# UCSC-VLAA/CLIPA

Measured on AMD Instinct MI355X. Metric: image-text pairs/sec (whole job), full training step, higher is better.
Workload: dtype bf16

## Files before the change

clipa_amd/csrc/attention.hip:

```cpp
#include "common.h"
#include "clipa_hip.h"
#include "attention_common.h"
#include "internal_hooks.h"

namespace {

template <int NKT, int DH, bool CAUSAL>
__global__ __launch_bounds__((64 * attn_waves<NKT, DH>()), HD<DH>::WGS) void attn_fwd_kernel(AttnArgs pin) {
  constexpr int LP = NKT * 32, RB = HD<DH>::RB, KS = HD<DH>::KS, DT = HD<DH>::DT;
  extern __shared__ __attribute__((aligned(16))) char smem[];
  constexpr int HPW = WGHeads<NKT>::HPW, WPH = attn_waves<NKT, DH>() / HPW;
  const int tid = threadIdx.x, lane = tid & 63;
  const int wave_wg = __builtin_amdgcn_readfirstlane(tid >> 6);
  const int slot = wave_wg / WPH, wave = wave_wg % WPH;
  char* sK = smem + slot * (2 * LP * RB);
  char* sV = sK + LP * RB;
  constexpr bool STAGE = fwd_stages<NKT, DH>();
  char* stage = smem + HPW * (2 * LP * RB) + wave_wg * Stg<DH>::BYTES;
  const int l31 = lane & 31, hi = lane >> 5, q16 = (lane >> 4) & 1, i16 = lane & 15;
  const long nheads = (long)pin.B * pin.H;
  const long head_raw = (long)blockIdx.x * HPW + slot;
  const bool live = head_raw < nheads;
  const long head = live ? head_raw : nheads - 1;
  const int b = (int)(head / pin.H), h = (int)(head - (long)b * pin.H);
  ATTN_LOCATE_SEQUENCE
  const size_t hoff = ((size_t)row0 * p.ld_qkv + (size_t)h * DH) * 2;
  const unsigned nrec = (unsigned)((long)(p.L - 1) * p.ld_qkv * 2 + DH * 2);
  const __amdgpu_buffer_rsrc_t rsQ = make_rsrc(p.q + hoff, nrec);
  const __amdgpu_buffer_rsrc_t rsK = make_rsrc(p.k + hoff, nrec);
  const __amdgpu_buffer_rsrc_t rsV = make_rsrc(p.v + hoff, nrec);
  dma_image<DH>(rsK, sK, LP, p.ld_qkv, wave, lane, WPH);
  dma_image<DH>(rsV, sV, LP, p.ld_qkv, wave, lane, WPH);
  constexpr bool PREFETCH = !(NKT == 9 && DH == 64);
  bf16x8 fq[KS], fqn[KS];
  if (PREFETCH) load_frags<KS, DH>(rsQ, p.ld_qkv, 32 * wave + l31, hi, fqn);
  asm volatile("s_waitcnt vmcnt(0)" ::: "memory");
  __syncthreads();

  for (int qt = wave; qt < NKT; qt += WPH) {
    const int qg = 32 * qt + l31;
    if (PREFETCH) {
#pragma unroll
      for (int ks = 0; ks < KS; ++ks) fq[ks] = fqn[ks];
      if (qt + WPH < NKT) load_frags<KS, DH>(rsQ, p.ld_qkv, qg + 32 * WPH, hi, fqn);
    } else {
      load_frags<KS, DH>(rsQ, p.ld_qkv, qg, hi, fq);
    }
    f32x16 s[NKT];
#pragma unroll
    for (int kt = 0; kt < NKT; ++kt) {
#pragma unroll
      for (int r = 0; r < 16; ++r) s[kt][r] = 0.f;
      if (CAUSAL && kt > qt) continue;
#pragma unroll
      for (int ks = 0; ks < KS; ++ks)
        s[kt] = __builtin_amdgcn_mfma_f32_32x32x16_bf16(frag_direct<DH>(sK, 32 * kt, l31, hi, ks), fq[ks], s[kt], 0, 0, 0);
      if (!CAUSAL && (kt & 1)) __builtin_amdgcn_sched_barrier(0);
    }
    float inv, m2;
    softmax_rows<NKT, CAUSAL>(s, p, qt, qg, hi, inv, m2);

    f32x16 o[DT];
#pragma unroll
    for (int dt = 0; dt < DT; ++dt)
#pragma unroll
      for (int r = 0; r < 16; ++r) o[dt][r] = 0.f;
#pragma unroll
    for (int kt = 0; kt < NKT; ++kt) {
      if (CAUSAL && kt > qt) continue;
#pragma unroll
      for (int s2 = 0; s2 < 2; ++s2) {
        float pv[8];
#pragma unroll
        for (int e = 0; e < 8; ++e) pv[e] = s[kt][8 * s2 + e];
        const bf16x8 pf = pack_frag(pv);
#pragma unroll
        for (int dt = 0; dt < DT; ++dt)
          o[dt] = __builtin_amdgcn_mfma_f32_32x32x16_bf16(frag_trans<DH>(sV, 32 * kt + 16 * s2, 32 * dt, hi, q16, i16), pf, o[dt], 0, 0, 0);
      }
    }
    if constexpr (STAGE) {
      if (live) store_tile<DH>(stage, p.o, p.ld_o, row0 + 32 * qt, p.L - 32 * qt, h * DH, lane, o, inv);
      if (qg < p.L && live && p.stats && hi == 0) *(float2*)(p.stats + (stat0 + qg) * 2) = make_float2(m2, inv);
    } else if (qg < p.L && live) {
#pragma unroll
      for (int dt = 0; dt < DT; ++dt)
        store_frag_T(p.o, p.ld_o, row0 + qg, h * DH + 32 * dt, hi, o[dt], inv, DH - 32 * dt);
      if (p.stats && hi == 0) *(float2*)(p.stats + (stat0 + qg) * 2) = make_float2(m2, inv);
    }
  }
}

template <int NKT, int DH, bool CAUSAL>
__global__ __launch_bounds__((64 * attn_waves<NKT, DH>()), HD<DH>::WGS) void attn_bwd_kernel(AttnArgs pin) {
  constexpr int LP = NKT * 32, RB = HD<DH>::RB, KS = HD<DH>::KS, DT = HD<DH>::DT;
  extern __shared__ __attribute__((aligned(16))) char smem[];
  constexpr int HPW = WGHeads<NKT>::HPW, WPH = attn_waves<NKT, DH>() / HPW;
  constexpr bool FENCE = DH == 80 && NKT >= 5;
  const int tid = threadIdx.x, lane = tid & 63;
  const int wave_wg = __builtin_amdgcn_readfirstlane(tid >> 6);
  const int slot = wave_wg / WPH, wave = wave_wg % WPH;
  char* img0 = smem + slot * (2 * LP * RB + 3 * LP * 4);
  char* img1 = img0 + LP * RB;
  float* sM = (float*)(img0 + 2 * LP * RB);
  float* sD = sM + 2 * LP;
  constexpr bool STAGE = bwd_stages<NKT, DH>();
  char* stage = smem + HPW * (2 * LP * RB + 3 * LP * 4) + wave_wg * Stg<DH>::BYTES;
  const int l31 = lane & 31, hi = lane >> 5, q16 = (lane >> 4) & 1, i16 = lane & 15;
  const long nheads = (long)pin.B * pin.H;
  const long head_raw = (long)blockIdx.x * HPW + slot;
  const bool live = head_raw < nheads;
  const long head = live ? head_raw : nheads - 1;
  const int b = (int)(head / pin.H), h = (int)(head - (long)b * pin.H);
  ATTN_LOCATE_SEQUENCE
  const size_t hoff = ((size_t)row0 * p.ld_qkv + (size_t)h * DH) * 2;
  const size_t ooff = ((size_t)row0 * p.ld_o + (size_t)h * DH) * 2;
  const unsigned nrec = (unsigned)((long)(p.L - 1) * p.ld_qkv * 2 + DH * 2);
  const unsigned nrec_o = (unsigned)((long)(p.L - 1) * p.ld_o * 2 + DH * 2);
  const __amdgpu_buffer_rsrc_t rsQ = make_rsrc(p.q + hoff, nrec), rsK = make_rsrc(p.k + hoff, nrec),
                               rsV = make_rsrc(p.v + hoff, nrec), rsDO = make_rsrc(p.d_o + ooff, nrec_o),
                               rsO = make_rsrc(p.o_in + ooff, nrec_o);
  const float c = p.scale * 1.4426950408889634f;
  const float* stats = p.stats + stat0 * 2;

  dma_image<DH>(rsK, img0, LP, p.ld_qkv, wave, lane, WPH);
  dma_image<DH>(rsV, img1, LP, p.ld_qkv, wave, lane, WPH);
  bf16x8 fq[KS], fdo[KS], fo[KS];
  load_frags<KS, DH>(rsQ, p.ld_qkv, 32 * wave + l31, hi, fq);
  load_frags<KS, DH>(rsDO, p.ld_o, 32 * wave + l31, hi, fdo);
  load_frags<KS, DH>(rsO, p.ld_o, 32 * wave + l31, hi, fo);
  asm volatile("s_waitcnt vmcnt(0)" ::: "memory");
  __syncthreads();
  for (int qt = wave; qt < NKT; qt += WPH) {
    const int qg = 32 * qt + l31;
    if (qt != wave) {
      load_frags<KS, DH>(rsQ, p.ld_qkv, qg, hi, fq);
      load_frags<KS, DH>(rsDO, p.ld_o, qg, hi, fdo);
      load_frags<KS, DH>(rsO, p.ld_o, qg, hi, fo);
    }
    float mp = 1e30f;
    if (qg < p.L) {
      const float2 st = *(const float2*)(stats + qg * 2);
      mp = st.x - __builtin_amdgcn_logf(st.y);
    }
    float Dq = 0.f;
#pragma unroll
    for (int ks = 0; ks < KS; ++ks) {
      float a[8], o8[8];
      unpack8(__builtin_bit_cast(u32x4, fdo[ks]), a);
      unpack8(__builtin_bit_cast(u32x4, fo[ks]), o8);
#pragma unroll
      for (int i = 0; i < 8; ++i) Dq += a[i] * o8[i];
    }
    Dq += __shfl_xor(Dq, 32, 64);
    if (hi == 0) { sM[qg] = mp; sD[qg] = Dq; }
    const int lim2 = (CAUSAL ? min(p.L, qg + 1) : p.L) - 4 * hi;
    f32x16 dq[DT];
#pragma unroll
    for (int dt = 0; dt < DT; ++dt)
#pragma unroll
      for (int r = 0; r < 16; ++r) dq[dt][r] = 0.f;
#pragma unroll
    for (int kt = 0; kt < NKT; ++kt) {
      if (CAUSAL && kt > qt) continue;
      f32x16 s, dp;
#pragma unroll
      for (int r = 0; r < 16; ++r) { s[r] = 0.f; dp[r] = 0.f; }
#pragma unroll
      for (int ks = 0; ks < KS; ++ks) {
        s = __builtin_amdgcn_mfma_f32_32x32x16_bf16(frag_direct<DH>(img0, 32 * kt, l31, hi, ks), fq[ks], s, 0, 0, 0);
        dp = __builtin_amdgcn_mfma_f32_32x32x16_bf16(frag_direct<DH>(img1, 32 * kt, l31, hi, ks), fdo[ks], dp, 0, 0, 0);
      }
      if constexpr (FENCE) __builtin_amdgcn_sched_barrier(0);
      const bool full = CAUSAL ? ((32 * kt + 32 <= p.L) && kt < qt) : (kt < NKT - 1);
      float ds[16];
#pragma unroll
      for (int r = 0; r < 16; ++r) {
        float pe = __builtin_amdgcn_exp2f(fmaf(s[r], c, -mp));
        if (!full) pe = (32 * kt + 8 * (r >> 2) + (r & 3) < lim2) ? pe : 0.f;
        ds[r] = pe * (dp[r] - Dq);
      }
      if constexpr (FENCE) __builtin_amdgcn_sched_barrier(0);
#pragma unroll
      for (int s2 = 0; s2 < 2; ++s2) {
        const bf16x8 dsf = pack_frag(ds + 8 * s2);
#pragma unroll
        for (int dt = 0; dt < DT; ++dt)
          dq[dt] = __builtin_amdgcn_mfma_f32_32x32x16_bf16(frag_trans<DH>(img0, 32 * kt + 16 * s2, 32 * dt, hi, q16, i16), dsf, dq[dt], 0, 0, 0);
      }
    }
    if constexpr (STAGE) {
      if (live) store_tile<DH>(stage, p.dq, p.ld_dqkv, row0 + 32 * qt, p.L - 32 * qt, h * DH, lane, dq, p.scale);
    } else if (qg < p.L && live) {
#pragma unroll
      for (int dt = 0; dt < DT; ++dt)
        store_frag_T(p.dq, p.ld_dqkv, row0 + qg, h * DH + 32 * dt, hi, dq[dt], p.scale, DH - 32 * dt);
    }
  }
  bf16x8 fk[KS], fv[KS];
#pragma unroll
  for (int ks = 0; ks < KS; ++ks) {
    fk[ks] = frag_direct<DH>(img0, 32 * min(wave, NKT - 1), l31, hi, ks);
    fv[ks] = frag_direct<DH>(img1, 32 * min(wave, NKT - 1), l31, hi, ks);
  }
  asm volatile("s_waitcnt lgkmcnt(0)" ::: "memory");
  __syncthreads();

  dma_image<DH>(rsQ, img0, LP, p.ld_qkv, wave, lane, WPH);
  dma_image<DH>(rsDO, img1, LP, p.ld_o, wave, lane, WPH);
  asm volatile("s_waitcnt vmcnt(0)" ::: "memory");
  __syncthreads();
  for (int kt = wave; kt < NKT; kt += WPH) {
    const int kg = 32 * kt + l31;
    const int kgc = l31 - 4 * hi;
    if (kt != wave) {
      load_frags<KS, DH>(rsK, p.ld_qkv, kg, hi, fk);
      load_frags<KS, DH>(rsV, p.ld_qkv, kg, hi, fv);
    }
    f32x16 dk[DT], dv[DT];
#pragma unroll
    for (int dt = 0; dt < DT; ++dt)
#pragma unroll
      for (int r = 0; r < 16; ++r) { dk[dt][r] = 0.f; dv[dt][r] = 0.f; }
    for (int qt = (CAUSAL ? kt : 0); qt < NKT; ++qt) {
      f32x16 s, dp;
#pragma unroll
      for (int r = 0; r < 16; ++r) { s[r] = 0.f; dp[r] = 0.f; }
#pragma unroll
      for (int ks = 0; ks < KS; ++ks) {
        s = __builtin_amdgcn_mfma_f32_32x32x16_bf16(frag_direct<DH>(img0, 32 * qt, l31, hi, ks), fk[ks], s, 0, 0, 0);
        dp = __builtin_amdgcn_mfma_f32_32x32x16_bf16(frag_direct<DH>(img1, 32 * qt, l31, hi, ks), fv[ks], dp, 0, 0, 0);
      }
      if constexpr (FENCE) __builtin_amdgcn_sched_barrier(0);
      float pr[16], ds[16];
#pragma unroll
      for (int rq = 0; rq < 4; ++rq) {
        const int q0 = 32 * qt + 8 * rq + 4 * hi;
        const float4 m4 = *(const float4*)(sM + q0);
        const float4 d4 = *(const float4*)(sD + q0);
        const float mm[4] = {m4.x, m4.y, m4.z, m4.w};
        const float dd[4] = {d4.x, d4.y, d4.z, d4.w};
#pragma unroll
        for (int e = 0; e < 4; ++e) {
          const int r = 4 * rq + e;
          float pe = __builtin_amdgcn_exp2f(fmaf(s[r], c, -mm[e]));
          if (CAUSAL && qt == kt) pe = (kgc <= 8 * rq + e) ? pe : 0.f;
          pr[r] = pe;
          ds[r] = pe * (dp[r] - dd[e]);
        }
      }
      if constexpr (FENCE) __builtin_amdgcn_sched_barrier(0);
#pragma unroll
      for (int s2 = 0; s2 < 2; ++s2) {
        const bf16x8 pf = pack_frag(pr + 8 * s2);
        const bf16x8 dsf = pack_frag(ds + 8 * s2);
#pragma unroll
        for (int dt = 0; dt < DT; ++dt) {
          dv[dt] = __builtin_amdgcn_mfma_f32_32x32x16_bf16(frag_trans<DH>(img1, 32 * qt + 16 * s2, 32 * dt, hi, q16, i16), pf, dv[dt], 0, 0, 0);
          dk[dt] = __builtin_amdgcn_mfma_f32_32x32x16_bf16(frag_trans<DH>(img0, 32 * qt + 16 * s2, 32 * dt, hi, q16, i16), dsf, dk[dt], 0, 0, 0);
        }
      }
    }
    if constexpr (STAGE) {
      if (live) {
        store_tile<DH>(stage, p.dk, p.ld_dqkv, row0 + 32 * kt, p.L - 32 * kt, h * DH, lane, dk, p.scale);
        store_tile<DH>(stage, p.dv, p.ld_dqkv, row0 + 32 * kt, p.L - 32 * kt, h * DH, lane, dv, 1.0f);
      }
    } else if (kg < p.L && live) {
#pragma unroll
      for (int dt = 0; dt < DT; ++dt) {
        store_frag_T(p.dk, p.ld_dqkv, row0 + kg, h * DH + 32 * dt, hi, dk[dt], p.scale, DH - 32 * dt);
        store_frag_T(p.dv, p.ld_dqkv, row0 + kg, h * DH + 32 * dt, hi, dv[dt], 1.0f, DH - 32 * dt);
      }
    }
  }
}

constexpr int LONG_CT = 8;
constexpr int LONG_LMAX = 1024;

template <int DH>
__device__ __forceinline__ __amdgpu_buffer_rsrc_t chunk_rsrc(const char* base, long ld, int row0, int L) {
  const long rows = (long)L - row0;
  const long bytes = rows > 0 ? (rows - 1) * ld * 2 + DH * 2 : 0;
  return make_rsrc(base + (size_t)row0 * ld * 2, (unsigned)bytes);
}

template <int DH, bool CAUSAL>
__global__ __launch_bounds__(256, HD<DH>::WGS) void attn_fwd_long_kernel(AttnArgs p) {
  constexpr int CT = LONG_CT, RB = HD<DH>::RB, KS = HD<DH>::KS, DT = HD<DH>::DT;
  extern __shared__ __attribute__((aligned(16))) char smem[];
  const int tid = threadIdx.x, lane = tid & 63;
  const int wave = __builtin_amdgcn_readfirstlane(tid >> 6);
  char* sK = smem;
  char* sV = sK + CT * 32 * RB;
  const int l31 = lane & 31, hi = lane >> 5, q16 = (lane >> 4) & 1, i16 = lane & 15;
  const long head = blockIdx.x;
  const int b = (int)(head / p.H), h = (int)(head - (long)b * p.H);
  const char* qb = p.q + ((size_t)b * p.L * p.ld_qkv + (size_t)h * DH) * 2;
  const char* kb = p.k + ((size_t)b * p.L * p.ld_qkv + (size_t)h * DH) * 2;
  const char* vb = p.v + ((size_t)b * p.L * p.ld_qkv + (size_t)h * DH) * 2;
  const __amdgpu_buffer_rsrc_t rsQ = chunk_rsrc<DH>(qb, p.ld_qkv, 0, p.L);
  const int NT = (p.L + 31) / 32;
  const float c = p.scale * 1.4426950408889634f;

  for (int qt0 = 0; qt0 < NT; qt0 += 4) {
    const int qt = qt0 + wave;
    const int qg = 32 * qt + l31;
    bf16x8 fq[KS];
    load_frags<KS, DH>(rsQ, p.ld_qkv, qg, hi, fq);
    const int lim2 = (CAUSAL ? min(p.L, qg + 1) : p.L) - 4 * hi;
    float m_run = -1e30f, l_run = 0.f;
    f32x16 o[DT];
#pragma unroll
    for (int dt = 0; dt < DT; ++dt)
#pragma unroll
      for (int r = 0; r < 16; ++r) o[dt][r] = 0.f;
    for (int kc = 0; kc < NT; kc += CT) {
      if (CAUSAL && kc > qt0 + 3) break;
      const int nct = min(CT, NT - kc);
      __syncthreads();
      dma_image<DH>(chunk_rsrc<DH>(kb, p.ld_qkv, 32 * kc, p.L), sK, nct * 32, p.ld_qkv, wave, lane, 4);
      dma_image<DH>(chunk_rsrc<DH>(vb, p.ld_qkv, 32 * kc, p.L), sV, nct * 32, p.ld_qkv, wave, lane, 4);
      asm volatile("s_waitcnt vmcnt(0)" ::: "memory");
      __syncthreads();
      f32x16 s[CT];
      float mx = -1e30f;
#pragma unroll
      for (int kt = 0; kt < CT; ++kt) {
#pragma unroll
        for (int r = 0; r < 16; ++r) s[kt][r] = 0.f;
        if (kt >= nct || (CAUSAL && kc + kt > qt)) continue;
#pragma unroll
        for (int ks = 0; ks < KS; ++ks)
          s[kt] = __builtin_amdgcn_mfma_f32_32x32x16_bf16(frag_direct<DH>(sK, 32 * kt, l31, hi, ks), fq[ks], s[kt], 0, 0, 0);
        const int T = kc + kt;
        const bool full = (32 * T + 32 <= p.L) && (!CAUSAL || T < qt);
#pragma unroll
        for (int r = 0; r < 16; ++r) {
          float v = s[kt][r];
          if (!full) v = (32 * T + 8 * (r >> 2) + (r & 3) < lim2) ? v : -1e30f;
          s[kt][r] = v;
          mx = fmaxf(mx, v);
        }
      }
      mx = fmaxf(mx, __shfl_xor(mx, 32, 64));
      const float m_new = fmaxf(m_run, mx);
      const float alpha = __builtin_amdgcn_exp2f((m_run - m_new) * c);
      const float m2 = m_new * c;
      float sum = 0.f;
#pragma unroll
      for (int kt = 0; kt < CT; ++kt) {
        if (kt >= nct || (CAUSAL && kc + kt > qt)) continue;
#pragma unroll
        for (int r = 0; r < 16; ++r) {
          const float v = s[kt][r];
          const float e = (v > -1e29f) ? __builtin_amdgcn_exp2f(fmaf(v, c, -m2)) : 0.f;
          s[kt][r] = e;
          sum += e;
        }
      }
      sum += __shfl_xor(sum, 32, 64);
      l_run = l_run * alpha + sum;
      m_run = m_new;
#pragma unroll
      for (int dt = 0; dt < DT; ++dt)
#pragma unroll
        for (int r = 0; r < 16; ++r) o[dt][r] *= alpha;
#pragma unroll
      for (int kt = 0; kt < CT; ++kt) {
        if (kt >= nct || (CAUSAL && kc + kt > qt)) continue;
#pragma unroll
        for (int s2 = 0; s2 < 2; ++s2) {
          float pv[8];
#pragma unroll
          for (int e = 0; e < 8; ++e) pv[e] = s[kt][8 * s2 + e];
          const bf16x8 pf = pack_frag(pv);
#pragma unroll
          for (int dt = 0; dt < DT; ++dt)
            o[dt] = __builtin_amdgcn_mfma_f32_32x32x16_bf16(frag_trans<DH>(sV, 32 * kt + 16 * s2, 32 * dt, hi, q16, i16), pf, o[dt], 0, 0, 0);
        }
      }
    }
    if (qg < p.L) {
      const float inv = 1.0f / l_run;
#pragma unroll
      for (int dt = 0; dt < DT; ++dt)
        store_frag_T(p.o, p.ld_o, (long)b * p.L + qg, h * DH + 32 * dt, hi, o[dt], inv, DH - 32 * dt);
      if (p.stats && hi == 0) *(float2*)(p.stats + ((size_t)head * p.L + qg) * 2) = make_float2(m_run * c, inv);
    }
  }
}

template <int DH, bool CAUSAL>
__global__ __launch_bounds__(256, HD<DH>::WGS) void attn_bwd_long_kernel(AttnArgs p) {
  constexpr int CT = LONG_CT, RB = HD<DH>::RB, KS = HD<DH>::KS, DT = HD<DH>::DT;
  extern __shared__ __attribute__((aligned(16))) char smem[];
  const int tid = threadIdx.x, lane = tid & 63;
  const int wave = __builtin_amdgcn_readfirstlane(tid >> 6);
  char* img0 = smem;
  char* img1 = img0 + CT * 32 * RB;
  float* sM = (float*)(img0 + 2 * CT * 32 * RB);
  float* sL = sM + LONG_LMAX;
  float* sD = sL + LONG_LMAX;
  const int l31 = lane & 31, hi = lane >> 5, q16 = (lane >> 4) & 1, i16 = lane & 15;
  const long head = blockIdx.x;
  const int b = (int)(head / p.H), h = (int)(head - (long)b * p.H);
  const size_t hoff = ((size_t)b * p.L * p.ld_qkv + (size_t)h * DH) * 2;
  const size_t ooff = ((size_t)b * p.L * p.ld_o + (size_t)h * DH) * 2;
  const __amdgpu_buffer_rsrc_t rsQ = chunk_rsrc<DH>(p.q + hoff, p.ld_qkv, 0, p.L), rsK = chunk_rsrc<DH>(p.k + hoff, p.ld_qkv, 0, p.L),
                               rsV = chunk_rsrc<DH>(p.v + hoff, p.ld_qkv, 0, p.L), rsDO = chunk_rsrc<DH>(p.d_o + ooff, p.ld_o, 0, p.L),
                               rsO = chunk_rsrc<DH>(p.o_in + ooff, p.ld_o, 0, p.L);
  const float c = p.scale * 1.4426950408889634f;
  const float* stats = p.stats + (size_t)head * p.L * 2;
  const int NT = (p.L + 31) / 32;

  for (int qt0 = 0; qt0 < NT; qt0 += 4) {
    const int qt = qt0 + wave;
    const int qg = 32 * qt + l31;
    bf16x8 fq[KS], fdo[KS], fo[KS];
    load_frags<KS, DH>(rsQ, p.ld_qkv, qg, hi, fq);
    load_frags<KS, DH>(rsDO, p.ld_o, qg, hi, fdo);
    load_frags<KS, DH>(rsO, p.ld_o, qg, hi, fo);
    float2 st = make_float2(0.f, 0.f);
    if (qg < p.L) st = *(const float2*)(stats + qg * 2);
    float Dq = 0.f;
#pragma unroll
    for (int ks = 0; ks < KS; ++ks) {
      float a[8], o8[8];
      unpack8(__builtin_bit_cast(u32x4, fdo[ks]), a);
      unpack8(__builtin_bit_cast(u32x4, fo[ks]), o8);
#pragma unroll
      for (int i = 0; i < 8; ++i) Dq += a[i] * o8[i];
    }
    Dq += __shfl_xor(Dq, 32, 64);
    if (hi == 0 && qt < NT) { sM[qg] = st.x; sL[qg] = st.y; sD[qg] = Dq; }
    const int lim2 = (CAUSAL ? min(p.L, qg + 1) : p.L) - 4 * hi;
    f32x16 dq[DT];
#pragma unroll
    for (int dt = 0; dt < DT; ++dt)
#pragma unroll
      for (int r = 0; r < 16; ++r) dq[dt][r] = 0.f;
    for (int kc = 0; kc < NT; kc += CT) {
      if (CAUSAL && kc > qt0 + 3) break;
      const int nct = min(CT, NT - kc);
      __syncthreads();
      dma_image<DH>(chunk_rsrc<DH>(p.k + hoff, p.ld_qkv, 32 * kc, p.L), img0, nct * 32, p.ld_qkv, wave, lane, 4);
      dma_image<DH>(chunk_rsrc<DH>(p.v + hoff, p.ld_qkv, 32 * kc, p.L), img1, nct * 32, p.ld_qkv, wave, lane, 4);
      asm volatile("s_waitcnt vmcnt(0)" ::: "memory");
      __syncthreads();
      for (int kt = 0; kt < nct; ++kt) {
        const int T = kc + kt;
        if (CAUSAL && T > qt) break;
        f32x16 s, dp;
#pragma unroll
        for (int r = 0; r < 16; ++r) { s[r] = 0.f; dp[r] = 0.f; }
#pragma unroll
        for (int ks = 0; ks < KS; ++ks) {
          s = __builtin_amdgcn_mfma_f32_32x32x16_bf16(frag_direct<DH>(img0, 32 * kt, l31, hi, ks), fq[ks], s, 0, 0, 0);
          dp = __builtin_amdgcn_mfma_f32_32x32x16_bf16(frag_direct<DH>(img1, 32 * kt, l31, hi, ks), fdo[ks], dp, 0, 0, 0);
        }
        const bool full = (32 * T + 32 <= p.L) && (!CAUSAL || T < qt);
        float ds[16];
#pragma unroll
        for (int r = 0; r < 16; ++r) {
          float pe = __builtin_amdgcn_exp2f(fmaf(s[r], c, -st.x)) * st.y;
          if (!full) pe = (32 * T + 8 * (r >> 2) + (r & 3) < lim2) ? pe : 0.f;
          ds[r] = pe * (dp[r] - Dq) * p.scale;
        }
#pragma unroll
        for (int s2 = 0; s2 < 2; ++s2) {
          const bf16x8 dsf = pack_frag(ds + 8 * s2);
#pragma unroll
          for (int dt = 0; dt < DT; ++dt)
            dq[dt] = __builtin_amdgcn_mfma_f32_32x32x16_bf16(frag_trans<DH>(img0, 32 * kt + 16 * s2, 32 * dt, hi, q16, i16), dsf, dq[dt], 0, 0, 0);
        }
      }
    }
    if (qg < p.L) {
#pragma unroll
      for (int dt = 0; dt < DT; ++dt)
        store_frag_T(p.dq, p.ld_dqkv, (long)b * p.L + qg, h * DH + 32 * dt, hi, dq[dt], 1.0f, DH - 32 * dt);
    }
  }

  for (int kt0 = 0; kt0 < NT; kt0 += 4) {
    const int kt = kt0 + wave;
    const int kg = 32 * kt + l31;
    const int kgc = l31 - 4 * hi;
    bf16x8 fk[KS], fv[KS];
    load_frags<KS, DH>(rsK, p.ld_qkv, kg, hi, fk);
    load_frags<KS, DH>(rsV, p.ld_qkv, kg, hi, fv);
    f32x16 dk[DT], dv[DT];
#pragma unroll
    for (int dt = 0; dt < DT; ++dt)
#pragma unroll
      for (int r = 0; r < 16; ++r) { dk[dt][r] = 0.f; dv[dt][r] = 0.f; }
    for (int qc = 0; qc < NT; qc += CT) {
      const int nct = min(CT, NT - qc);
      if (CAUSAL && qc + nct <= kt0) continue;
      __syncthreads();
      dma_image<DH>(chunk_rsrc<DH>(p.q + hoff, p.ld_qkv, 32 * qc, p.L), img0, nct * 32, p.ld_qkv, wave, lane, 4);
      dma_image<DH>(chunk_rsrc<DH>(p.d_o + ooff, p.ld_o, 32 * qc, p.L), img1, nct * 32, p.ld_o, wave, lane, 4);
      asm volatile("s_waitcnt vmcnt(0)" ::: "memory");
      __syncthreads();
      for (int qi = 0; qi < nct; ++qi) {
        const int T = qc + qi;
        if (CAUSAL && T < kt) continue;
        f32x16 s, dp;
#pragma unroll
        for (int r = 0; r < 16; ++r) { s[r] = 0.f; dp[r] = 0.f; }
#pragma unroll
        for (int ks = 0; ks < KS; ++ks) {
          s = __builtin_amdgcn_mfma_f32_32x32x16_bf16(frag_direct<DH>(img0, 32 * qi, l31, hi, ks), fk[ks], s, 0, 0, 0);
          dp = __builtin_amdgcn_mfma_f32_32x32x16_bf16(frag_direct<DH>(img1, 32 * qi, l31, hi, ks), fv[ks], dp, 0, 0, 0);
        }
        float pr[16], ds[16];
#pragma unroll
        for (int rq = 0; rq < 4; ++rq) {
          const int q0 = 32 * T + 8 * rq + 4 * hi;
          const float4 m4 = *(const float4*)(sM + q0);
          const float4 l4 = *(const float4*)(sL + q0);
          const float4 d4 = *(const float4*)(sD + q0);
          const float mm[4] = {m4.x, m4.y, m4.z, m4.w};
          const float ll[4] = {l4.x, l4.y, l4.z, l4.w};
          const float dd[4] = {d4.x, d4.y, d4.z, d4.w};
#pragma unroll
          for (int e = 0; e < 4; ++e) {
            const int r = 4 * rq + e;
            float pe = __builtin_amdgcn_exp2f(fmaf(s[r], c, -mm[e])) * ll[e];
            if (CAUSAL && T == kt) pe = (kgc <= 8 * rq + e) ? pe : 0.f;
            pr[r] = pe;
            ds[r] = pe * (dp[r] - dd[e]) * p.scale;
          }
        }
#pragma unroll
        for (int s2 = 0; s2 < 2; ++s2) {
          const bf16x8 pf = pack_frag(pr + 8 * s2);
          const bf16x8 dsf = pack_frag(ds + 8 * s2);
#pragma unroll
          for (int dt = 0; dt < DT; ++dt) {
            dv[dt] = __builtin_amdgcn_mfma_f32_32x32x16_bf16(frag_trans<DH>(img1, 32 * qi + 16 * s2, 32 * dt, hi, q16, i16), pf, dv[dt], 0, 0, 0);
            dk[dt] = __builtin_amdgcn_mfma_f32_32x32x16_bf16(frag_trans<DH>(img0, 32 * qi + 16 * s2, 32 * dt, hi, q16, i16), dsf, dk[dt], 0, 0, 0);
          }
        }
      }
    }
    if (kg < p.L) {
#pragma unroll
      for (int dt = 0; dt < DT; ++dt) {
        store_frag_T(p.dk, p.ld_dqkv, (long)b * p.L + kg, h * DH + 32 * dt, hi, dk[dt], 1.0f, DH - 32 * dt);
        store_frag_T(p.dv, p.ld_dqkv, (long)b * p.L + kg, h * DH + 32 * dt, hi, dv[dt], 1.0f, DH - 32 * dt);
      }
    }
  }
}

template <int NKT, int DH, bool CAUSAL>
int launch_fwd_c(const AttnArgs& a, hipStream_t st) {
  constexpr int HPW = WGHeads<NKT>::HPW;
  const int lds = HPW * 2 * NKT * 32 * HD<DH>::RB + (fwd_stages<NKT, DH>() ? attn_waves<NKT, DH>() * Stg<DH>::BYTES : 0);
  static clipa_gemm::LdsOptIn optin;
  int dev = 0;
  if (int rc = clipa_gemm::current_device(&dev)) return rc;
  if (int rc = optin.ensure(dev, {(const void*)attn_fwd_kernel<NKT, DH, CAUSAL>}, lds, "attn_fwd")) return rc;
  hipLaunchKernelGGL((attn_fwd_kernel<NKT, DH, CAUSAL>), dim3((unsigned)(((long)a.B * a.H + HPW - 1) / HPW)), dim3(64 * attn_waves<NKT, DH>()), lds, st, a);
  return clipa_check_launch("attn_fwd");
}
template <int NKT, int DH>
int launch_fwd(const AttnArgs& a, hipStream_t st) {
  return a.causal ? launch_fwd_c<NKT, DH, true>(a, st) : launch_fwd_c<NKT, DH, false>(a, st);
}
template <int NKT, int DH, bool CAUSAL>
int launch_bwd_c(const AttnArgs& a, hipStream_t st) {
  constexpr int HPW = WGHeads<NKT>::HPW;
  const int lds = HPW * (2 * NKT * 32 * HD<DH>::RB + 3 * NKT * 32 * 4) + (bwd_stages<NKT, DH>() ? attn_waves<NKT, DH>() * Stg<DH>::BYTES : 0);
  static clipa_gemm::LdsOptIn optin;
  int dev = 0;
  if (int rc = clipa_gemm::current_device(&dev)) return rc;
  if (int rc = optin.ensure(dev, {(const void*)attn_bwd_kernel<NKT, DH, CAUSAL>}, lds, "attn_bwd")) return rc;
  hipLaunchKernelGGL((attn_bwd_kernel<NKT, DH, CAUSAL>), dim3((unsigned)(((long)a.B * a.H + HPW - 1) / HPW)), dim3(64 * attn_waves<NKT, DH>()), lds, st, a);
  return clipa_check_launch("attn_bwd");
}
template <int NKT, int DH>
int launch_bwd(const AttnArgs& a, hipStream_t st) {
  return a.causal ? launch_bwd_c<NKT, DH, true>(a, st) : launch_bwd_c<NKT, DH, false>(a, st);
}

template <int DH, bool CAUSAL, bool BWD>
int launch_long(const AttnArgs& a, hipStream_t st) {
  const int lds = 2 * LONG_CT * 32 * HD<DH>::RB + (BWD ? 3 * LONG_LMAX * 4 : 0);
  const void* fn = BWD ? (const void*)attn_bwd_long_kernel<DH, CAUSAL> : (const void*)attn_fwd_long_kernel<DH, CAUSAL>;
  static clipa_gemm::LdsOptIn optin;
  int dev = 0;
  if (int rc = clipa_gemm::current_device(&dev)) return rc;
  if (int rc = optin.ensure(dev, {fn}, lds, "attention (long)")) return rc;
  const dim3 grid((unsigned)((long)a.B * a.H));
  if (BWD) hipLaunchKernelGGL((attn_bwd_long_kernel<DH, CAUSAL>), grid, dim3(256), lds, st, a);
  else hipLaunchKernelGGL((attn_fwd_long_kernel<DH, CAUSAL>), grid, dim3(256), lds, st, a);
  return clipa_check_launch(BWD ? "attn_bwd_long" : "attn_fwd_long");
}
#ifndef CLIPA_ATTN_WIDE
template <bool BWD>
int dispatch_long(const AttnArgs& a, int64_t dh, hipStream_t st) {
  if (dh == 80) return a.causal ? launch_long<80, true, BWD>(a, st) : launch_long<80, false, BWD>(a, st);
  return a.causal ? launch_long<64, true, BWD>(a, st) : launch_long<64, false, BWD>(a, st);
}
#endif

bool wide_head(int64_t dh) { return dh == 88 || dh == 104 || dh == 112; }

int check_args(int64_t B, int64_t H, int64_t L, int64_t dh, int64_t ld_qkv, int64_t ld_o, int causal) {
  if (dh != 64 && dh != 80 && !wide_head(dh)) { clipa_set_error("attention: head dim %ld unsupported (64, 80, 88, 104, 112)", (long)dh); return CLIPA_ERR_ARG; }
  if (wide_head(dh) && causal) { clipa_set_error("attention: head dim %ld is compiled for image towers only (no causal mask)", (long)dh); return CLIPA_ERR_ARG; }
  if (L <= 0 || L > LONG_LMAX) { clipa_set_error("attention: L=%ld outside (0, %d]", (long)L, LONG_LMAX); return CLIPA_ERR_ARG; }
  if (ld_qkv % 8 != 0 || ld_o % 8 != 0) { clipa_set_error("attention: row strides must be multiples of 8 elements"); return CLIPA_ERR_ARG; }
  if (B * H <= 0 || B * H > 0x7fffffffL) { clipa_set_error("attention: bad B*H"); return CLIPA_ERR_ARG; }
  return 0;
}

}

#define ATTN_DISPATCH_DH(fn, DH, a, st)                                     \
  switch (((a).L + 31) / 32) {                                               \
    case 1: return fn<1, DH>(a, st); case 2: return fn<2, DH>(a, st);        \
    case 3: return fn<3, DH>(a, st); case 4: return fn<4, DH>(a, st);        \
    case 5: return fn<5, DH>(a, st); case 6: return fn<6, DH>(a, st);        \
    case 7: return fn<7, DH>(a, st); case 8: return fn<8, DH>(a, st);        \
    default: return fn<9, DH>(a, st);                                        \
  }
#ifdef CLIPA_ATTN_WIDE
template <int NKT, int DH> int wide_fwd(const AttnArgs& a, hipStream_t st) { return launch_fwd_c<NKT, DH, false>(a, st); }
template <int NKT, int DH> int wide_bwd(const AttnArgs& a, hipStream_t st) { return launch_bwd_c<NKT, DH, false>(a, st); }
template <int DH>
int wide_dh(const AttnArgs& a, int bwd, hipStream_t st) {
  if (a.L > 288) return bwd ? launch_long<DH, false, true>(a, st) : launch_long<DH, false, false>(a, st);
  if (bwd) { ATTN_DISPATCH_DH(wide_bwd, DH, a, st) }
  ATTN_DISPATCH_DH(wide_fwd, DH, a, st)
}
extern "C" int clipa_attn_wide_launch(const void* args, int64_t dh, int bwd, void* stream) {
  const AttnArgs& a = *(const AttnArgs*)args;
  if (dh == 88) return wide_dh<88>(a, bwd, (hipStream_t)stream);
  if (dh == 104) return wide_dh<104>(a, bwd, (hipStream_t)stream);
  return wide_dh<112>(a, bwd, (hipStream_t)stream);
}
#else
extern "C" int clipa_attn_wide_launch(const void* args, int64_t dh, int bwd, void* stream);
#ifdef CLIPA_ATTN_PERSISTENT_EXPERIMENT
extern "C" int clipa_attn_bwd1_try(const void* args, int64_t dh, void* stream, int* rc);
extern "C" int clipa_attn_fwd1_try(const void* args, int64_t dh, void* stream, int* rc);
#endif

#define ATTN_DISPATCH(fn, dh, a, st)                 \
  if ((dh) == 80) { ATTN_DISPATCH_DH(fn, 80, a, st) } \
  ATTN_DISPATCH_DH(fn, 64, a, st)

extern "C" int clipa_attention_fwd(const void* q, const void* k, const void* v, void* out, float* stats,
                                   int64_t B, int64_t H, int64_t L, int64_t dh, int64_t ld_qkv, int64_t ld_o,
                                   float scale, int causal, void* stream) {
  if (B * H == 0) return CLIPA_OK;
  if (int rc = check_args(B, H, L, dh, ld_qkv, ld_o, causal)) return rc;
  AttnArgs a = {};
  a.q = (const char*)q; a.k = (const char*)k; a.v = (const char*)v; a.ld_qkv = ld_qkv;
  a.o = (char*)out; a.ld_o = ld_o; a.B = (int)B; a.H = (int)H; a.L = (int)L; a.scale = scale; a.causal = causal;
  a.stats = stats;
  if (wide_head(dh)) return clipa_attn_wide_launch(&a, dh, 0, stream);
  if (L > 288) return dispatch_long<false>(a, dh, (hipStream_t)stream);
#ifdef CLIPA_ATTN_PERSISTENT_EXPERIMENT
  int rc1 = 0;
  if ((clipa_internal_debug_flags() & 524288) && clipa_attn_fwd1_try(&a, dh, stream, &rc1)) return rc1;
#endif
  ATTN_DISPATCH(launch_fwd, dh, a, (hipStream_t)stream)
}

extern "C" int clipa_attention_bwd(const void* q, const void* k, const void* v, const void* out,
                                   const void* d_out, const float* stats, void* dq, void* dk, void* dv, int64_t B, int64_t H,
                                   int64_t L, int64_t dh, int64_t ld_qkv, int64_t ld_o, int64_t ld_dqkv,
                                   float scale, int causal, void* stream) {
  if (B * H == 0) return CLIPA_OK;
  if (int rc = check_args(B, H, L, dh, ld_qkv, ld_o, causal)) return rc;
  if (ld_dqkv % 8 != 0) { clipa_set_error("attention_bwd: ld_dqkv must be a multiple of 8"); return CLIPA_ERR_ARG; }
  if (!stats) { clipa_set_error("attention_bwd: needs the forward's softmax statistics"); return CLIPA_ERR_ARG; }
  AttnArgs a = {};
  a.q = (const char*)q; a.k = (const char*)k; a.v = (const char*)v; a.ld_qkv = ld_qkv;
  a.o_in = (const char*)out; a.d_o = (const char*)d_out; a.ld_o = ld_o;
  a.dq = (char*)dq; a.dk = (char*)dk; a.dv = (char*)dv; a.ld_dqkv = ld_dqkv;
  a.B = (int)B; a.H = (int)H; a.L = (int)L; a.scale = scale; a.causal = causal;
  a.stats = const_cast<float*>(stats);
  if (wide_head(dh)) return clipa_attn_wide_launch(&a, dh, 1, stream);
  if (L > 288) return dispatch_long<true>(a, dh, (hipStream_t)stream);
#ifdef CLIPA_ATTN_PERSISTENT_EXPERIMENT
  int rc1 = 0;
  if ((clipa_internal_debug_flags() & 262144) && clipa_attn_bwd1_try(&a, dh, stream, &rc1)) return rc1;
#endif
  ATTN_DISPATCH(launch_bwd, dh, a, (hipStream_t)stream)
}
namespace {
int varlen_args(const int* seq_start, const int* seq_len, int64_t nseq, int64_t tiles, int64_t dh) {
  if (!seq_start || !seq_len) { clipa_set_error("attention (varlen): seq_start / seq_len missing"); return CLIPA_ERR_ARG; }
  if (tiles < 1 || tiles > 9) { clipa_set_error("attention (varlen): tiles=%ld outside [1, 9] (sequences of up to 288 tokens)", (long)tiles); return CLIPA_ERR_ARG; }
  if (dh != 64 && dh != 80) { clipa_set_error("attention (varlen): head dim %ld unsupported (64 and 80)", (long)dh); return CLIPA_ERR_ARG; }
  (void)nseq;
  return 0;
}
}

extern "C" int clipa_attention_fwd_varlen(const void* q, const void* k, const void* v, void* out, float* stats,
                                          const int32_t* seq_start, const int32_t* seq_len, const int32_t* seq_ids, int64_t nseq,
                                          int64_t tiles, int64_t H, int64_t dh, int64_t ld_qkv, int64_t ld_o, float scale,
                                          int causal, void* stream) {
  if (nseq * H == 0) return CLIPA_OK;
  if (int rc = check_args(nseq, H, 32 * tiles, dh, ld_qkv, ld_o, causal)) return rc;
  if (int rc = varlen_args(seq_start, seq_len, nseq, tiles, dh)) return rc;
  AttnArgs a = {};
  a.q = (const char*)q; a.k = (const char*)k; a.v = (const char*)v; a.ld_qkv = ld_qkv;
  a.o = (char*)out; a.ld_o = ld_o; a.B = (int)nseq; a.H = (int)H; a.L = (int)(32 * tiles); a.scale = scale; a.causal = causal;
  a.stats = stats;
  a.seq_start = seq_start; a.seq_len = seq_len; a.seq_ids = seq_ids;
  ATTN_DISPATCH(launch_fwd, dh, a, (hipStream_t)stream)
}

extern "C" int clipa_attention_bwd_varlen(const void* q, const void* k, const void* v, const void* out, const void* d_out,
                                          const float* stats, void* dq, void* dk, void* dv, const int32_t* seq_start,
                                          const int32_t* seq_len, const int32_t* seq_ids, int64_t nseq, int64_t tiles, int64_t H,
                                          int64_t dh, int64_t ld_qkv, int64_t ld_o, int64_t ld_dqkv, float scale, int causal,
                                          void* stream) {
  if (nseq * H == 0) return CLIPA_OK;
  if (int rc = check_args(nseq, H, 32 * tiles, dh, ld_qkv, ld_o, causal)) return rc;
  if (int rc = varlen_args(seq_start, seq_len, nseq, tiles, dh)) return rc;
  if (ld_dqkv % 8 != 0) { clipa_set_error("attention_bwd (varlen): ld_dqkv must be a multiple of 8"); return CLIPA_ERR_ARG; }
  if (!stats) { clipa_set_error("attention_bwd (varlen): needs the forward's softmax statistics"); return CLIPA_ERR_ARG; }
  AttnArgs a = {};
  a.q = (const char*)q; a.k = (const char*)k; a.v = (const char*)v; a.ld_qkv = ld_qkv;
  a.o_in = (const char*)out; a.d_o = (const char*)d_out; a.ld_o = ld_o;
  a.dq = (char*)dq; a.dk = (char*)dk; a.dv = (char*)dv; a.ld_dqkv = ld_dqkv;
  a.B = (int)nseq; a.H = (int)H; a.L = (int)(32 * tiles); a.scale = scale; a.causal = causal;
  a.stats = const_cast<float*>(stats);
  a.seq_start = seq_start; a.seq_len = seq_len; a.seq_ids = seq_ids;
  ATTN_DISPATCH(launch_bwd, dh, a, (hipStream_t)stream)
}
#endif
```

clipa_amd/csrc/attention_common.h:

```cpp
#pragma once
#include "common.h"

namespace {

struct AttnArgs {
  const char* q; const char* k; const char* v; long ld_qkv;
  char* o; const char* o_in; const char* d_o; long ld_o;
  char* dq; char* dk; char* dv; long ld_dqkv;
  float* stats;
  int B, H, L;
  float scale;
  int causal;
  const int* seq_start; const int* seq_len; const int* seq_ids;
  int abl;
};

template <int DH>
struct HD {
  static constexpr int RB = DH == 64 ? 128 : 256;
  static constexpr int NCH = RB / 16;
  static constexpr int KS = (DH + 15) / 16;
  static constexpr int DT = (DH + 31) / 32;
  static constexpr int WGS = DH == 64 ? 2 : 1;
};
template <int NKT>
struct WGHeads {
  static constexpr int HPW = NKT == 1 ? 4 : (NKT == 2 ? 2 : 1);
  static constexpr int WPH = 4 / HPW;
};
template <int NKT, int DH>
__host__ __device__ constexpr int attn_waves() { return (DH == 80 && NKT >= 5) ? 8 : 4; }

template <int DH>
__device__ __forceinline__ int swz_u(int row) {
  if (DH == 64) return (((row >> 1) & 1) << 2) | ((row >> 2) & 1) | (((row >> 3) & 1) << 1);
  return ((row & 3) << 2) | ((row >> 2) & 3);
}

template <int DH>
__device__ __forceinline__ void dma_image(const __amdgpu_buffer_rsrc_t rs, char* img, int LP, long ld,
                                          int wave, int lane, int nwaves = 4) {
  constexpr int NCH = HD<DH>::NCH, RPP = 1024 / HD<DH>::RB;
  for (int pc = wave; pc < LP / RPP; pc += nwaves) {
    const int row = pc * RPP + lane / NCH;
    const int chunk = (lane & (NCH - 1)) ^ swz_u<DH>(row);
    const unsigned oob = (chunk * 8 >= DH) ? 0x80000000u : 0u;
    __builtin_amdgcn_raw_ptr_buffer_load_lds(rs, LDS_PTR(img + pc * 1024), 16,
                                             (unsigned)(row * ld * 2 + chunk * 16) | oob, 0, 0, 0);
  }
}

template <int DH>
__device__ __forceinline__ bf16x8 frag_direct(const char* img, int rowbase, int l31, int hi, int ks) {
  return *(const bf16x8*)(img + (rowbase + l31) * HD<DH>::RB + (((2 * ks + hi) ^ swz_u<DH>(l31)) << 4));
}

template <int DH>
__device__ __forceinline__ bf16x8 frag_trans(const char* img, int rowbase16, int colbase, int hi, int q16, int i16) {
  constexpr int RB = HD<DH>::RB;
  const int col = colbase + 16 * q16 + 4 * (i16 & 3);
  const int r0 = rowbase16 + 4 * hi + (i16 >> 2);
  const int r1 = r0 + 8;
  const bf16x4 a = __builtin_amdgcn_ds_read_tr16_b64_v4i16(
      (__attribute__((address_space(3))) bf16x4*)(img + r0 * RB + (((col >> 3) ^ swz_u<DH>(r0)) << 4) + (col & 7) * 2));
  const bf16x4 b = __builtin_amdgcn_ds_read_tr16_b64_v4i16(
      (__attribute__((address_space(3))) bf16x4*)(img + r1 * RB + (((col >> 3) ^ swz_u<DH>(r1)) << 4) + (col & 7) * 2));
  bf16x8 f;
  f[0] = a[0]; f[1] = a[1]; f[2] = a[2]; f[3] = a[3];
  f[4] = b[0]; f[5] = b[1]; f[6] = b[2]; f[7] = b[3];
  return f;
}

__device__ __forceinline__ bf16x8 pack_frag(const float* v) {
  u32x4 w;
#pragma unroll
  for (int i = 0; i < 4; ++i) w[i] = pack2bf(v[2 * i], v[2 * i + 1]);
  return __builtin_bit_cast(bf16x8, w);
}

__device__ __forceinline__ void store_frag_T(char* base, long ld, long row, int col0, int hi, const f32x16& a, float mul,
                                             int ncols = 32) {
#pragma unroll
  for (int qd = 0; qd < 4; ++qd) {
    if (8 * qd >= ncols) continue;
    u32x2 w;
    w[0] = pack2bf(a[4 * qd + 0] * mul, a[4 * qd + 1] * mul);
    w[1] = pack2bf(a[4 * qd + 2] * mul, a[4 * qd + 3] * mul);
    *(u32x2*)(base + (row * ld + col0 + 8 * qd + 4 * hi) * 2) = w;
  }
}

__device__ __forceinline__ void store_tile64(char* stage, char* base, long ld, long row0, int rows_valid, int col0, int lane,
                                             const f32x16& a0, const f32x16& a1, float mul) {
  const int l31 = lane & 31, hi = lane >> 5;
#pragma unroll
  for (int dt = 0; dt < 2; ++dt) {
    const f32x16& a = dt ? a1 : a0;
#pragma unroll
    for (int qd = 0; qd < 4; ++qd) {
      u32x2 w;
      w[0] = pack2bf(a[4 * qd + 0] * mul, a[4 * qd + 1] * mul);
      w[1] = pack2bf(a[4 * qd + 2] * mul, a[4 * qd + 3] * mul);
      *(u32x2*)(stage + l31 * 128 + (((4 * dt + qd) ^ (l31 & 7)) << 4) + 8 * hi) = w;
    }
  }
  asm volatile("s_waitcnt lgkmcnt(0)" ::: "memory");
  const int chunk = lane & 7;
#pragma unroll
  for (int j = 0; j < 4; ++j) {
    const int row = 8 * j + (lane >> 3);
    const u32x4 v = *(const u32x4*)(stage + row * 128 + ((chunk ^ (row & 7)) << 4));
    if (row < rows_valid) *(u32x4*)(base + ((row0 + row) * ld + col0) * 2 + chunk * 16) = v;
  }
  asm volatile("" ::: "memory");
}

__device__ __forceinline__ void store_tile80(char* stage, char* base, long ld, long row0, int rows_valid, int col0, int lane,
                                             const f32x16& a0, const f32x16& a1, const f32x16& a2, float mul) {
  const int l31 = lane & 31, hi = lane >> 5;
#pragma unroll
  for (int h = 0; h < 2; ++h) {
    if ((l31 >> 4) == h) {
#pragma unroll
      for (int dt = 0; dt < 3; ++dt) {
        const f32x16& a = dt == 0 ? a0 : (dt == 1 ? a1 : a2);
#pragma unroll
        for (int qd = 0; qd < 4; ++qd) {
          if (4 * dt + qd >= 10) continue;
          u32x2 w;
          w[0] = pack2bf(a[4 * qd + 0] * mul, a[4 * qd + 1] * mul);
          w[1] = pack2bf(a[4 * qd + 2] * mul, a[4 * qd + 3] * mul);
          *(u32x2*)(stage + (l31 & 15) * 160 + (4 * dt + qd) * 16 + 8 * hi) = w;
        }
      }
    }
    asm volatile("s_waitcnt lgkmcnt(0)" ::: "memory");
#pragma unroll
    for (int j = 0; j < 3; ++j) {
      const int task = 64 * j + lane;
      if (task < 160) {
        const u32x4 v = *(const u32x4*)(stage + task * 16);
        const int row = task / 10, chunk = task - 10 * row;
        if (16 * h + row < rows_valid) *(u32x4*)(base + ((row0 + 16 * h + row) * ld + col0) * 2 + chunk * 16) = v;
      }
    }
    asm volatile("s_waitcnt lgkmcnt(0)" ::: "memory");
  }
}
template <int DH>
struct Stg { static constexpr int BYTES = DH == 64 ? 4096 : 2560; };
template <int DH>
__device__ __forceinline__ void store_tile(char* stage, char* base, long ld, long row0, int rows_valid, int col0, int lane,
                                           const f32x16* a, float mul) {
  if constexpr (DH == 64) store_tile64(stage, base, ld, row0, rows_valid, col0, lane, a[0], a[1], mul);
  else store_tile80(stage, base, ld, row0, rows_valid, col0, lane, a[0], a[1], a[2], mul);
}

template <int NKT, bool CAUSAL>
__device__ __forceinline__ void softmax_rows(f32x16 (&s)[NKT], const AttnArgs& p, int qt, int qg, int hi,
                                             float& inv, float& m2) {
  const float c = p.scale * 1.4426950408889634f;
  const int lim2 = (CAUSAL ? min(p.L, qg + 1) : p.L) - 4 * hi;
  float mx = -1e30f;
#pragma unroll
  for (int kt = 0; kt < NKT; ++kt) {
    const bool full = CAUSAL ? ((32 * kt + 32 <= p.L) && kt < qt) : (kt < NKT - 1);
#pragma unroll
    for (int r = 0; r < 16; ++r) {
      float v = s[kt][r];
      if (!full) v = (32 * kt + 8 * (r >> 2) + (r & 3) < lim2) ? v : -1e30f;
      s[kt][r] = v;
      mx = fmaxf(mx, v);
    }
  }
  mx = fmaxf(mx, __shfl_xor(mx, 32, 64));
  m2 = mx * c;
  float sum = 0.f;
#pragma unroll
  for (int kt = 0; kt < NKT; ++kt)
#pragma unroll
    for (int r = 0; r < 16; ++r) {
      const float e = __builtin_amdgcn_exp2f(fmaf(s[kt][r], c, -m2));
      s[kt][r] = e;
      sum += e;
    }
  sum += __shfl_xor(sum, 32, 64);
  inv = 1.0f / sum;
}

template <int KS, int DH>
__device__ __forceinline__ void load_frags(const __amdgpu_buffer_rsrc_t rs, long ld, int row, int hi, bf16x8 (&f)[KS]) {
#pragma unroll
  for (int ks = 0; ks < KS; ++ks) {
    const unsigned oob = ((2 * ks + hi) * 8 >= DH) ? 0x80000000u : 0u;
    f[ks] = __builtin_bit_cast(bf16x8, __builtin_amdgcn_raw_buffer_load_b128(rs, (unsigned)(row * ld * 2 + (2 * ks + hi) * 16) | oob, 0, 0));
  }
}

template <int NKT, int DH>
__host__ __device__ constexpr bool fwd_stages() {
  return (DH == 64 || DH == 80) && (WGHeads<NKT>::HPW * 2 * NKT * 32 * HD<DH>::RB + attn_waves<NKT, DH>() * Stg<DH>::BYTES) * HD<DH>::WGS <= 160 * 1024;
}
template <int NKT, int DH>
__host__ __device__ constexpr bool bwd_stages() {
  return (DH == 64 || DH == 80) && (WGHeads<NKT>::HPW * (2 * NKT * 32 * HD<DH>::RB + 3 * NKT * 32 * 4) + attn_waves<NKT, DH>() * Stg<DH>::BYTES) * HD<DH>::WGS <= 160 * 1024;
}

#define ATTN_LOCATE_SEQUENCE                                                     \
  AttnArgs p = pin;                                                              \
  long row0 = (long)b * pin.L;                                                   \
  size_t stat0 = (size_t)head * pin.L;                                           \
  if (pin.seq_len) {                                                             \
    const int sid = pin.seq_ids ? pin.seq_ids[b] : b;                            \
    p.L = pin.seq_len[sid];                                                      \
    row0 = pin.seq_start[sid];                                                   \
    stat0 = (size_t)row0 * pin.H + (size_t)h * p.L;                              \
  }

}
```

Baseline: 2465.

## Rebuild Q/dO LDS images from register fragments in attention backward

In the attention backward kernel, the Q and dO LDS images for the dK/dV phase are rebuilt from fragments the waves already hold in registers, replacing a second global DMA of those tensors. Likewise, the K/V fragments for a wave's second tile are read from the existing LDS image instead of reloaded from global memory. This trades global memory traffic and a vmcnt wait for extra registers holding a spare fragment set. It is gated per configuration by a constexpr table excluding some NKT/DH/causal cases, and only applies when each wave handles at most two tiles.

```diff
diff --git a/clipa_amd/csrc/attention.hip b/clipa_amd/csrc/attention.hip
--- a/clipa_amd/csrc/attention.hip
+++ b/clipa_amd/csrc/attention.hip
@@ -97,7 +97,10 @@
   extern __shared__ __attribute__((aligned(16))) char smem[];
   constexpr int HPW = WGHeads<NKT>::HPW, WPH = attn_waves<NKT, DH>() / HPW;
   constexpr bool FENCE = DH == 80 && NKT >= 5;
-  const int tid = threadIdx.x, lane = tid & 63;
+  constexpr bool REBUILD = bwd_rebuild<NKT, DH, CAUSAL>();
+  static_assert(!REBUILD || bwd_tiles_per_wave<NKT, DH>() <= 2, "one spare fragment set: at most two tiles per wave");
+  const int tid = threadIdx.x;
+  int lane = tid & 63;
   const int wave_wg = __builtin_amdgcn_readfirstlane(tid >> 6);
   const int slot = wave_wg / WPH, wave = wave_wg % WPH;
   char* img0 = smem + slot * (2 * LP * RB + 3 * LP * 4);
@@ -106,7 +109,7 @@
   float* sD = sM + 2 * LP;
   constexpr bool STAGE = bwd_stages<NKT, DH>();
   char* stage = smem + HPW * (2 * LP * RB + 3 * LP * 4) + wave_wg * Stg<DH>::BYTES;
-  const int l31 = lane & 31, hi = lane >> 5, q16 = (lane >> 4) & 1, i16 = lane & 15;
+  int l31 = lane & 31, hi = lane >> 5, q16 = (lane >> 4) & 1, i16 = lane & 15;
   const long nheads = (long)pin.B * pin.H;
   const long head_raw = (long)blockIdx.x * HPW + slot;
   const bool live = head_raw < nheads;
@@ -126,6 +129,7 @@
   dma_image<DH>(rsK, img0, LP, p.ld_qkv, wave, lane, WPH);
   dma_image<DH>(rsV, img1, LP, p.ld_qkv, wave, lane, WPH);
   bf16x8 fq[KS], fdo[KS], fo[KS];
+  bf16x8 fq0[KS], fdo0[KS];
   load_frags<KS, DH>(rsQ, p.ld_qkv, 32 * wave + l31, hi, fq);
   load_frags<KS, DH>(rsDO, p.ld_o, 32 * wave + l31, hi, fdo);
   load_frags<KS, DH>(rsO, p.ld_o, 32 * wave + l31, hi, fo);
@@ -134,6 +138,10 @@
   for (int qt = wave; qt < NKT; qt += WPH) {
     const int qg = 32 * qt + l31;
     if (qt != wave) {
+      if constexpr (REBUILD) {
+#pragma unroll
+        for (int ks = 0; ks < KS; ++ks) { fq0[ks] = fq[ks]; fdo0[ks] = fdo[ks]; }
+      }
       load_frags<KS, DH>(rsQ, p.ld_qkv, qg, hi, fq);
       load_frags<KS, DH>(rsDO, p.ld_o, qg, hi, fdo);
       load_frags<KS, DH>(rsO, p.ld_o, qg, hi, fo);
@@ -197,25 +205,61 @@
         store_frag_T(p.dq, p.ld_dqkv, row0 + qg, h * DH + 32 * dt, hi, dq[dt], p.scale, DH - 32 * dt);
     }
   }
-  bf16x8 fk[KS], fv[KS];
+  const bool two = bwd_tiles_per_wave<NKT, DH>() == 2 && wave + WPH < NKT;
+  bf16x8 fk[KS], fv[KS], fk1[KS], fv1[KS];
 #pragma unroll
   for (int ks = 0; ks < KS; ++ks) {
     fk[ks] = frag_direct<DH>(img0, 32 * min(wave, NKT - 1), l31, hi, ks);
     fv[ks] = frag_direct<DH>(img1, 32 * min(wave, NKT - 1), l31, hi, ks);
   }
+  if constexpr (REBUILD) {
+    if (two) {
+#pragma unroll
+      for (int ks = 0; ks < KS; ++ks) {
+        fk1[ks] = frag_direct<DH>(img0, 32 * (wave + WPH), l31, hi, ks);
+        fv1[ks] = frag_direct<DH>(img1, 32 * (wave + WPH), l31, hi, ks);
+      }
+    }
+  }
   asm volatile("s_waitcnt lgkmcnt(0)" ::: "memory");
   __syncthreads();
 
-  dma_image<DH>(rsQ, img0, LP, p.ld_qkv, wave, lane, WPH);
-  dma_image<DH>(rsDO, img1, LP, p.ld_o, wave, lane, WPH);
-  asm volatile("s_waitcnt vmcnt(0)" ::: "memory");
+  if constexpr (REBUILD) {
+    lane = __builtin_amdgcn_mbcnt_hi(~0u, __builtin_amdgcn_mbcnt_lo(~0u, 0u));
+    l31 = lane & 31, hi = lane >> 5, q16 = (lane >> 4) & 1, i16 = lane & 15;
+    if (two) {
+#pragma unroll
+      for (int ks = 0; ks < KS; ++ks) {
+        frag_store_direct<DH>(img0, 32 * wave, l31, hi, ks, fq0[ks]);
+        frag_store_direct<DH>(img1, 32 * wave, l31, hi, ks, fdo0[ks]);
+      }
+    }
+    if (wave < NKT) {
+      const int last = two ? wave + WPH : wave;
+#pragma unroll
+      for (int ks = 0; ks < KS; ++ks) {
+        frag_store_direct<DH>(img0, 32 * last, l31, hi, ks, fq[ks]);
+        frag_store_direct<DH>(img1, 32 * last, l31, hi, ks, fdo[ks]);
+      }
+    }
+    asm volatile("s_waitcnt lgkmcnt(0)" ::: "memory");
+  } else {
+    dma_image<DH>(rsQ, img0, LP, p.ld_qkv, wave, lane, WPH);
+    dma_image<DH>(rsDO, img1, LP, p.ld_o, wave, lane, WPH);
+    asm volatile("s_waitcnt vmcnt(0)" ::: "memory");
+  }
   __syncthreads();
   for (int kt = wave; kt < NKT; kt += WPH) {
     const int kg = 32 * kt + l31;
     const int kgc = l31 - 4 * hi;
     if (kt != wave) {
-      load_frags<KS, DH>(rsK, p.ld_qkv, kg, hi, fk);
-      load_frags<KS, DH>(rsV, p.ld_qkv, kg, hi, fv);
+      if constexpr (REBUILD) {
+#pragma unroll
+        for (int ks = 0; ks < KS; ++ks) { fk[ks] = fk1[ks]; fv[ks] = fv1[ks]; }
+      } else {
+        load_frags<KS, DH>(rsK, p.ld_qkv, kg, hi, fk);
+        load_frags<KS, DH>(rsV, p.ld_qkv, kg, hi, fv);
+      }
     }
     f32x16 dk[DT], dv[DT];
 #pragma unroll
diff --git a/clipa_amd/csrc/attention_common.h b/clipa_amd/csrc/attention_common.h
--- a/clipa_amd/csrc/attention_common.h
+++ b/clipa_amd/csrc/attention_common.h
@@ -53,6 +53,11 @@
 template <int DH>
 __device__ __forceinline__ bf16x8 frag_direct(const char* img, int rowbase, int l31, int hi, int ks) {
   return *(const bf16x8*)(img + (rowbase + l31) * HD<DH>::RB + (((2 * ks + hi) ^ swz_u<DH>(l31)) << 4));
+}
+
+template <int DH>
+__device__ __forceinline__ void frag_store_direct(char* img, int rowbase, int l31, int hi, int ks, const bf16x8& f) {
+  *(bf16x8*)(img + (rowbase + l31) * HD<DH>::RB + (((2 * ks + hi) ^ swz_u<DH>(l31)) << 4)) = f;
 }
 
 template <int DH>
@@ -206,6 +211,18 @@
   return (DH == 64 || DH == 80) && (WGHeads<NKT>::HPW * (2 * NKT * 32 * HD<DH>::RB + 3 * NKT * 32 * 4) + attn_waves<NKT, DH>() * Stg<DH>::BYTES) * HD<DH>::WGS <= 160 * 1024;
 }
 
+template <int NKT, int DH>
+__host__ __device__ constexpr int bwd_tiles_per_wave() {
+  constexpr int WPH = attn_waves<NKT, DH>() / WGHeads<NKT>::HPW;
+  return (NKT + WPH - 1) / WPH;
+}
+template <int NKT, int DH, bool CAUSAL>
+__host__ __device__ constexpr bool bwd_rebuild() {
+  if (DH == 64 && !CAUSAL && (NKT == 3 || NKT == 5 || NKT == 8)) return false;
+  if (DH == 80 && ((CAUSAL && NKT == 9) || (!CAUSAL && NKT == 2))) return false;
+  return bwd_tiles_per_wave<NKT, DH>() <= 2 && DH <= 80;
+}
+
 #define ATTN_LOCATE_SEQUENCE                                                     \
   AttnArgs p = pin;                                                              \
   long row0 = (long)b * pin.L;                                                   \
```

Measured after the change: 2473, median of 6. About the same (+0.3%).
